# decadenza/SimpleStereo

Hardware: AMD Instinct MI355X
Metric: disparity MPixels/s (H*W*nDisp per second) (higher is better)
Workload: dtype f32

## Files before the change

### include/ssamd.h

```cpp
#ifndef SSAMD_H
#define SSAMD_H

#include <stdint.h>

#ifdef __cplusplus
extern "C" {
#endif

#define SSAMD_ABI_VERSION 8

#define SSAMD_OK 0
#define SSAMD_EINVAL (-1)
#define SSAMD_ENODEVICE (-2)
#define SSAMD_EHIP (-3)
#define SSAMD_ENOMEM (-4)
#define SSAMD_ELIMIT (-5)

int ssamd_abi_version(void);
const char *ssamd_last_error(void);
int ssamd_device_count(void);


int ssamd_asw(const uint8_t *img1, const uint8_t *img2, int height, int width,
              int winSize, int maxDisparity, int minDisparity,
// ... 83 lines not shown
                               int height, int width, int interpolation, int winSize, int maxDisparity, int minDisparity,
                               double gammaC, double gammaP, int consistent, int16_t *d_disparity, void *stream);

int ssamd_asw_exact_rectified_device(const uint8_t *d_raw1, const uint8_t *d_raw2, int src_height, int src_width,
                                     const float *d_mapx1, const float *d_mapy1, const float *d_mapx2, const float *d_mapy2,
                                     int height, int width, int interpolation, int winSize, int maxDisparity, int minDisparity,
                                     double gammaC, double gammaP, int consistent, int16_t *d_disparity, void *stream);

int ssamd_gsw_rectified_device(const uint8_t *d_raw1, const uint8_t *d_raw2, int src_height, int src_width,
                               const float *d_mapx1, const float *d_mapy1, const float *d_mapx2, const float *d_mapy2,
                               int height, int width, int interpolation, int winSize, int maxDisparity, int minDisparity,
                               int gamma, float fMax, int iterations, int bins, int16_t *d_disparity, void *stream);

int ssamd_reproject_device(const int16_t *d_disparity, int h, int w, const double *Q, float *d_points, void *stream);

int ssamd_iir_unwrap(const double *phase, int n, int h, int w, double tau, double *out, int device);
int ssamd_iir_unwrap_device(const double *d_phase, int n, int h, int w, double tau, double *d_out, void *stream);

int ssamd_np_unwrap(const double *p, long long outer, long long len, long long inner, double discont, double period, double *out,
                    int device);
int ssamd_np_unwrap_device(const double *d_p, long long outer, long long len, long long inner, double discont, double period,
                           double *d_out, void *stream);
int ssamd_np_unwrap_xy(const double *p, int n, int h, int w, double *out, int device);
int ssamd_np_unwrap_xy_device(const double *d_p, int n, int h, int w, double *d_out, void *stream);
int ssamd_np_unwrap_plan(long long outer, long long len, long long inner, int32_t *plan);

#define SSAMD_FTP_MAX_W 8192
int ssamd_ftp_phase(const uint8_t *img_obj, int ch_obj, const uint8_t *img_ref, int ch_ref, int h, int w, const double *fmin,
                    const double *fmax, int unwrap, double tau, double *out, int device);
int ssamd_ftp_phase_device(const uint8_t *d_img_obj, int ch_obj, const uint8_t *d_img_ref, int ch_ref, int h, int w,
                           const double *fmin, const double *fmax, int unwrap, double tau, double *d_out, void *stream);
int ssamd_ftp_band(int w, int h, const double *fmin, const double *fmax, int32_t *slo, int32_t *shi);


int ssamd_asw_costs(const uint8_t *img1, const uint8_t *img2, int height, int width,
                    int winSize, int maxDisparity, int minDisparity,
                    double gammaC, double gammaP, float *costs, int device);

int ssamd_asw_argmins(const uint8_t *img1, const uint8_t *img2, int height, int width,
                      int winSize, int maxDisparity, int minDisparity,
                      double gammaC, double gammaP,
                      int16_t *left_disparity, int16_t *right_match, int device);

int ssamd_bgr2lab(const uint8_t *img, int height, int width, float *lab, int device);

int ssamd_debug_libm(int which, int n, const void *in, void *out);
int ssamd_debug_exact_queue(int which, long long max_n, unsigned long long *entries, unsigned int *keys, long long *n);

int ssamd_debug_exact_costs(const uint8_t *img1, const uint8_t *img2, int height, int width, int winSize, double gammaC, double gammaP,
                            int n, const int *yxd, double *costs, double *lab1, double *lab2);

int ssamd_debug_gsw_sqrt(int n, float *out);

#define SSAMD_K_LAB 0
#define SSAMD_K_ASW_AGG 1
#define SSAMD_K_ASW_FIN 2
#define SSAMD_K_GSW_AGG 3
#define SSAMD_K_GSW_FIN 4
#define SSAMD_K_REMAP 5
#define SSAMD_K_REPROJECT 6
#define SSAMD_K_ASW_ALT 7
#define SSAMD_K_ASW_EXACT 8
#define SSAMD_K_UNWRAP 9
#define SSAMD_K_FTP 10
#define SSAMD_K_NPUNWRAP 11
#define SSAMD_K_COUNT 12
int ssamd_profile_enable(int on);
int ssamd_profile_reset(void);
int ssamd_profile_read(double *ms , long long *launches );
const char *ssamd_kernel_name(int slot);

int ssamd_set_option(const char *name, const char *value);

int ssamd_counter(int device, const char *name, long long *value);

int ssamd_autotune(int on);

int ssamd_asw_geometry(int width, int rows, int winSize, int maxDisparity, int minDisparity, int *out);

int ssamd_asw_kernel_form(int width, int rows, int winSize, int maxDisparity, int minDisparity, int *out);

int ssamd_gsw_geometry(int width, int rows, int winSize, int maxDisparity, int minDisparity, int *out);

#ifdef __cplusplus
}
#endif
#endif
```

### simplestereo_amd/_native.py

```python
import ctypes
import os

from .build import LIB_PATH as _DEFAULT_LIB_PATH

LIB_PATH = _DEFAULT_LIB_PATH
if os.environ.get("SSAMD_LIB"):
    if os.environ.get("SSAMD_EXPERIMENT") != "1":
        raise ImportError("SSAMD_LIB is an experiment hook: set SSAMD_EXPERIMENT=1 as well to load %s instead of the product "
                          "library" % os.environ["SSAMD_LIB"])
    LIB_PATH = os.environ["SSAMD_LIB"]
ABI_VERSION = 8

(K_LAB, K_ASW_AGG, K_ASW_FIN, K_GSW_AGG, K_GSW_FIN, K_REMAP, K_REPROJECT, K_ASW_ALT, K_ASW_EXACT, K_UNWRAP, K_FTP,
 K_NPUNWRAP, K_COUNT) = 0, 1, 2, 3, 4, 5, 6, 7, 8, 9, 10, 11, 12

_lib = None
_u8p = ctypes.c_void_p
_i16p = ctypes.c_void_p


class NativeError(RuntimeError):

    def __init__(self, code, msg):
        super().__init__("libssamd error %d: %s" % (code, msg))
# ... 46 lines not shown
    L.ssamd_gsw_device_rows2.restype = I
    L.ssamd_gsw_device_rows2.argtypes = [P, P, I, I, I, I, I, I, I, I, I, I, F, I, I, P, P]
    L.ssamd_asw_exact_device_rows2.restype = I
    L.ssamd_asw_exact_device_rows2.argtypes = [P, P, I, I, I, I, I, I, I, I, I, D, D, I, P, P]
    L.ssamd_asw_exact_rectified_device.restype = I
    L.ssamd_asw_exact_rectified_device.argtypes = [P, P, I, I, P, P, P, P, I, I, I, I, I, I, D, D, I, P, P]
    L.ssamd_asw_alternate.restype = I
    L.ssamd_asw_alternate.argtypes = [P, P, I, I, I, I, I, D, D, I, P, I]
    L.ssamd_asw_alternate_device.restype = I
    L.ssamd_asw_alternate_device.argtypes = [P, P, I, I, I, I, I, D, D, I, P, P]
    L.ssamd_asw_alternate_rows_device.restype = I
    L.ssamd_asw_alternate_rows_device.argtypes = [P, P, I, I, I, I, I, I, I, I, D, D, I, P, P]
    L.ssamd_asw_alternate_multi.restype = I
    L.ssamd_asw_alternate_multi.argtypes = [P, P, I, I, I, I, I, D, D, I, P, ctypes.POINTER(I), I]
    L.ssamd_asw_costs.restype = I
    L.ssamd_asw_costs.argtypes = [P, P, I, I, I, I, I, D, D, P, I]
    L.ssamd_asw_argmins.restype = I
    L.ssamd_asw_argmins.argtypes = [P, P, I, I, I, I, I, D, D, P, P, I]
    L.ssamd_bgr2lab.restype = I
    L.ssamd_bgr2lab.argtypes = [P, I, I, P, I]
    L.ssamd_remap_bgr_device.restype = I
    L.ssamd_remap_bgr_device.argtypes = [P, I, I, P, P, I, I, I, P, P]
    L.ssamd_reproject_device.restype = I
    L.ssamd_reproject_device.argtypes = [P, I, I, ctypes.POINTER(D), P, P]
    L.ssamd_iir_unwrap.restype = I
    L.ssamd_iir_unwrap.argtypes = [P, I, I, I, D, P, I]
    L.ssamd_iir_unwrap_device.restype = I
    L.ssamd_iir_unwrap_device.argtypes = [P, I, I, I, D, P, P]
    L.ssamd_ftp_phase.restype = I
    L.ssamd_ftp_phase.argtypes = [P, I, P, I, I, I, P, P, I, D, P, I]
    L.ssamd_ftp_phase_device.restype = I
    L.ssamd_ftp_phase_device.argtypes = [P, I, P, I, I, I, P, P, I, D, P, P]
    L.ssamd_ftp_band.restype = I
    L.ssamd_ftp_band.argtypes = [I, I, P, P, P, P]
    LL = ctypes.c_longlong
    L.ssamd_np_unwrap.restype = I
    L.ssamd_np_unwrap.argtypes = [P, LL, LL, LL, D, D, P, I]
    L.ssamd_np_unwrap_device.restype = I
    L.ssamd_np_unwrap_device.argtypes = [P, LL, LL, LL, D, D, P, P]
    L.ssamd_np_unwrap_xy.restype = I
    L.ssamd_np_unwrap_xy.argtypes = [P, I, I, I, P, I]
    L.ssamd_np_unwrap_xy_device.restype = I
    L.ssamd_np_unwrap_xy_device.argtypes = [P, I, I, I, P, P]
    L.ssamd_np_unwrap_plan.restype = I
    L.ssamd_np_unwrap_plan.argtypes = [LL, LL, LL, ctypes.POINTER(ctypes.c_int32)]
    L.ssamd_debug_exact_queue.restype = I
    L.ssamd_debug_exact_queue.argtypes = [I, ctypes.c_longlong, P, P, P]
    L.ssamd_debug_libm.restype = I
    L.ssamd_debug_libm.argtypes = [I, I, P, P]
    L.ssamd_debug_exact_costs.restype = I
    L.ssamd_debug_exact_costs.argtypes = [P, P, I, I, I, D, D, I, P, P, P, P]
    L.ssamd_debug_gsw_sqrt.restype = I
    L.ssamd_debug_gsw_sqrt.argtypes = [I, P]
    L.ssamd_profile_enable.restype = I
    L.ssamd_profile_enable.argtypes = [I]
    L.ssamd_profile_reset.restype = I
    L.ssamd_profile_read.restype = I
    L.ssamd_profile_read.argtypes = [ctypes.POINTER(D), ctypes.POINTER(ctypes.c_longlong)]
    L.ssamd_kernel_name.restype = ctypes.c_char_p
    L.ssamd_kernel_name.argtypes = [I]
    L.ssamd_autotune.restype = I
    L.ssamd_autotune.argtypes = [I]
    L.ssamd_asw_geometry.restype = I
    L.ssamd_asw_geometry.argtypes = [I, I, I, I, I, ctypes.POINTER(I)]
    L.ssamd_asw_kernel_form.restype = I
    L.ssamd_asw_kernel_form.argtypes = [I, I, I, I, I, ctypes.POINTER(I)]
    L.ssamd_gsw_geometry.restype = I
    L.ssamd_gsw_geometry.argtypes = [I, I, I, I, I, ctypes.POINTER(I)]
    L.ssamd_set_option.restype = I
    L.ssamd_set_option.argtypes = [ctypes.c_char_p, ctypes.c_char_p]
    L.ssamd_asw_rectified_device.restype = I
    L.ssamd_asw_rectified_device.argtypes = [P, P, I, I, P, P, P, P, I, I, I, I, I, I, D, D, I, P, P]
    L.ssamd_gsw_rectified_device.restype = I
    L.ssamd_gsw_rectified_device.argtypes = [P, P, I, I, P, P, P, P, I, I, I, I, I, I, I, F, I, I, P, P]
    L.ssamd_counter.restype = I
    L.ssamd_counter.argtypes = [I, ctypes.c_char_p, ctypes.POINTER(ctypes.c_longlong)]
    _lib = L
    return L


def set_option(name, value):
    check(lib().ssamd_set_option(name.encode(), None if value is None else str(value).encode()))


def counter(name, device=-1):
    v = ctypes.c_longlong(0)
    check(lib().ssamd_counter(device, name.encode(), ctypes.byref(v)))
    return int(v.value)


class options:

    def __init__(self, **kw):
        self.kw = kw

    def __enter__(self):
        done = []
        try:
            for k, v in self.kw.items():
                set_option(k, v)
                done.append(k)
        except Exception:
            for k in done:
                set_option(k, None)
            raise
        return self
# ... 47 lines not shown
```

### simplestereo_amd/csrc/asw_kernels.hip.h

```cpp
#pragma once
#include "common.hip.h"

namespace ssamd {

static constexpr int ASW_RX = 8;
static constexpr int ASW_RD = 4;
static constexpr int ASW_WB = 4;
static constexpr int ASW_MAX_THREADS = 768;
__host__ __device__ constexpr int asw_nwr(int rx) { return (rx + ASW_RD - 1 + 3) / 4 * 4; }
static_assert(ASW_RD == 4 && asw_nwr(8) == 12 && asw_nwr(4) == 8, "the main loop is unrolled for 8x4 and 4x4 register tiles");

struct AswGeom {
    int Tx, XG, DG, Dc, nchunks, threads;
    int Rx;
    int nL, nR, nRc, SR, Se, emask;
    int SL, hL, hR;
    int wseg, wlen;
    int JC;
    int e2;
    int e_bytes;
    int pipe;
    int NC, JCmax;
    int dephase;
    int wave_rx;
    int off_wL, off_wR, off_e, off_labL, off_labR, off_bgrL, off_bgrR, off_bestL, off_bestR, off_cen, off_prox;
    int lds_bytes;
    int lds_bytes_evol;
};

struct AswExactQueue {
    u64 *entries;
    uint32_t *ekeys;
    unsigned int *counter;
    unsigned char *flagL, *flagR;
    unsigned char *zeroL, *zeroR;
    unsigned char *zrow;
    unsigned int W;
    unsigned int cap;
    uint32_t tol;
    float sat_abs;
    uint32_t deep;
};

struct AswArgs {
    const PixRec *recL, *recR;
    const float *prox;
    u64 *keyL;
    u64 *keyR;
    int16_t *disp;
    const unsigned char *evol;
    int erow0, erows, evolW;
    float *costs;
    int cost_keys;
    int H, W, win, pad, minD, maxD, row0, rows;
    int ystep;
    int yb0;
    int yskip_at, yskip;
    float kC;
    AswExactQueue xq;
    AswGeom g;
    unsigned int *pq;
    int pq_nx, pq_ny, pq_items;
};
static constexpr int ASW_PQ_QUEUES = 8;
static constexpr int ASW_PQ_LINE = 32;

struct AswPipeTileId { int win, XG, DG, JC; };
__host__ __device__ constexpr int asw_cx_round_up(int v, int m) { return (v + m - 1) / m * m; }
__host__ __device__ constexpr int asw_cx_max(int a, int b) { return a > b ? a : b; }
__host__ __device__ constexpr AswGeom asw_pipe_geom_constexpr(AswPipeTileId t)
{
    AswGeom g{};
    const int win = t.win, p = win / 2;
    g.Rx = 8; g.JC = t.JC; g.pipe = 1; g.wave_rx = 0; g.e2 = 1; g.nchunks = 1;
    g.NC = (win + t.JC / 2) / t.JC;
    g.JCmax = asw_cx_max(t.JC, win - (g.NC - 1) * t.JC);
    g.XG = t.XG; g.DG = t.DG;
    g.Tx = 8 * t.XG; g.Dc = ASW_RD * t.DG;
    g.threads = asw_cx_round_up(t.XG * t.DG, 64);
    g.dephase = g.threads / 64 >= 12 ? 1 : 0;
    g.nL = g.Tx + 2 * p;
    g.nRc = g.Tx + g.Dc - 1;
    g.nR = g.nRc + 2 * p;
    g.hL = 0; g.hR = 0;
    g.SL = asw_cx_round_up(g.Tx, 4);
    g.SR = asw_cx_round_up(g.nRc + 1, 4);
    g.Se = 16 * ((t.DG + 3) / 4);
    g.emask = 0;
    const int wrows = 2 * g.JCmax;
    int off = 0;
    g.off_wL = off; off = (off + wrows * g.SL * 4 + 15) & ~15;
    g.off_wR = off; off = (off + wrows * g.SR * 4 + 15) & ~15;
    g.e_bytes = (g.nL * g.Se + 15) & ~15;
    g.off_e = off; off = (off + g.e_bytes * 2 + 15) & ~15;
    g.off_labL = off; off = (off + g.nL * 16 * 2 + 15) & ~15;
    g.off_labR = off; off = (off + g.nR * 16 * 2 + 15) & ~15;
    g.off_bestL = off; off = (off + g.Tx * 8 + 15) & ~15;
    g.off_bestR = off; off = (off + (g.nRc + 1) * 8 + 15) & ~15;
    g.off_cen = off; off = (off + (g.Tx + g.nRc) * 16 + 15) & ~15;
    g.off_prox = off; off = (off + win * 4 * 2 + 15) & ~15;
    g.lds_bytes_evol = off;
    g.off_bgrL = off; off = (off + g.nL * 4 * 2 + 15) & ~15;
    g.off_bgrR = off; off = (off + g.nR * 4 * 2 + 15) & ~15;
    g.lds_bytes = off;
    return g;
}
template <int SLC, int SRC, int SEC> struct AswPipeTile { static constexpr AswPipeTileId id{35, 1, 1, 16}; };
template <> struct AswPipeTile<120, 316, 208> { static constexpr AswPipeTileId id{35, 15, 49, 16}; };
template <> struct AswPipeTile<88, 348, 272> { static constexpr AswPipeTileId id{35, 11, 65, 16}; };
template <> struct AswPipeTile<216, 284, 80> { static constexpr AswPipeTileId id{35, 27, 17, 16}; };
inline bool asw_pipe_geom_matches(const AswGeom &a, const AswGeom &b)
{
    return a.pipe == b.pipe && a.Rx == b.Rx && a.JC == b.JC && a.NC == b.NC && a.JCmax == b.JCmax && a.XG == b.XG && a.DG == b.DG && a.Tx == b.Tx &&
           a.Dc == b.Dc && a.threads == b.threads && a.dephase == b.dephase && a.nL == b.nL && a.nRc == b.nRc && a.nR == b.nR && a.SL == b.SL &&
           a.SR == b.SR && a.Se == b.Se && a.e_bytes == b.e_bytes && a.off_wL == b.off_wL && a.off_wR == b.off_wR && a.off_e == b.off_e &&
// ... 577 lines not shown
```

### simplestereo_amd/csrc/asw_pipe_kernel.hip.h

```cpp
#pragma once
#include "asw_kernels.hip.h"
#ifndef SSAMD_KERNEL_TU
#include "lab_kernels.hip.h"
#endif

namespace ssamd {

#ifndef SSAMD_KERNEL_TU
static constexpr int TADV_COLS = 64;
template <bool BYTES>
__device__ __forceinline__ void asw_tad_tile(const void *__restrict__ srcL, const void *__restrict__ srcR, unsigned char *__restrict__ evol,
                                             int W, int pad, int minD, int Dc, int Se, int erow0, int erows, int evolW, int rd, long long npix_total,
                                             int bx, int by, int bz, char *smem)
{
    uint32_t *const sL = reinterpret_cast<uint32_t *>(smem);
    uint32_t *const sR = sL + TADV_COLS;
    const int r = erow0 + by, z = bz, uc0 = bx * TADV_COLS;
    const int P = Se >> 2, dlo = minD + z * Dc, dhi = dlo + Dc - 1;
    const int u0 = uc0 - pad, xr0 = u0 - dhi;
    auto pixel = [&](const void *src, int col) -> uint32_t {
        const size_t q = (size_t)r * W + col;
        if constexpr (BYTES) {
            typedef uint32_t __attribute__((aligned(1))) u32_unaligned;
            const uint8_t *const b = reinterpret_cast<const uint8_t *>(src) + 3 * q;
            return (long long)q + 1 < npix_total ? (*reinterpret_cast<const u32_unaligned *>(b) & 0xffffffu)
                                                 : ((uint32_t)b[0] | ((uint32_t)b[1] << 8) | ((uint32_t)b[2] << 16));
        } else {
            return reinterpret_cast<const PixRec *>(src)[q].bgrx;
        }
    };
    for (int k = threadIdx.x; k < 2 * TADV_COLS + Dc; k += blockDim.x) {
        const bool isL = k < TADV_COLS;
        const int col = isL ? u0 + k : xr0 + (k - TADV_COLS);
        const uint32_t v = (unsigned)col < (unsigned)W ? pixel(isL ? srcL : srcR, col) : 0x80000000u;
        (isL ? sL : sR)[isL ? k : k - TADV_COLS] = v;
    }
    __syncthreads();
    const int ncols = min(TADV_COLS, evolW - uc0);
    uint32_t *const out = reinterpret_cast<uint32_t *>(evol + (((size_t)z * erows + by) * (size_t)evolW + uc0) * Se);
    auto dword = [&](int c, int slot, uint32_t lp) {
        uint32_t v = 0;
        const int d0 = rd == 6 ? 6 * (slot >> 1) + 4 * (slot & 1) : 4 * slot, nv = rd == 6 && (slot & 1) ? 2 : 4;
        if (!(lp >> 31) && d0 < Dc) {
            const uint32_t *const rp = sR + c + (Dc - 1) - d0;
#pragma unroll
            for (int q = 0; q < 4; ++q) {
                const uint32_t rv = q < nv && d0 + q < Dc ? rp[-q] : 0x80000000u;
                if (!(rv >> 31)) v |= min(__builtin_amdgcn_sad_u8(lp, rv, 0u), 40u) << (8 * q);
            }
        }
        return v;
    };
    if ((P & 3) == 0) {
        const int P4 = P >> 2;
// ... 62 lines not shown

template <bool WITH_COSTS, int SLC = 0, int SRC = 0, int SEC = 0, bool CG = false>
__global__ __launch_bounds__(ASW_MAX_THREADS, 3) void asw_aggregate_pipe_kernel(const AswArgs A0)
{
    constexpr bool STATIC = SLC > 0;
    static_assert(!CG || STATIC, "compile-time geometry belongs to a static tile");
    constexpr int RX = ASW_RX;
    constexpr int NWR = asw_nwr(RX);
    extern __shared__ __attribute__((aligned(16))) char smem[];
    constexpr AswGeom SG = asw_pipe_geom_constexpr(AswPipeTile<SLC, SRC, SEC>::id);
    static_assert(!STATIC || (SG.SL == SLC && SG.SR == SRC && SG.Se == SEC), "the strides name the tile");
    uint32_t *const pq_next = reinterpret_cast<uint32_t *>(smem + (CG ? SG : A0.g).off_prox);
    int pq_q = 0;
    auto run_item = [&](const AswArgs &A, const int ibx, const int iby, const int ibz, const int inx) __attribute__((always_inline)) {
    const bool persist = A.pq != nullptr;
    const AswGeom &g = CG ? SG : A.g;
    float *const wL = reinterpret_cast<float *>(smem + g.off_wL);
    float *const wR = reinterpret_cast<float *>(smem + g.off_wR);
    unsigned char *const eT0 = reinterpret_cast<unsigned char *>(smem + g.off_e);
    float4 *const labL = reinterpret_cast<float4 *>(smem + g.off_labL);
    float4 *const labR = reinterpret_cast<float4 *>(smem + g.off_labR);
    uint32_t *const bgrL = reinterpret_cast<uint32_t *>(smem + g.off_bgrL);
    uint32_t *const bgrR = reinterpret_cast<uint32_t *>(smem + g.off_bgrR);
    u64 *const bestL = reinterpret_cast<u64 *>(smem + g.off_bestL);
    u64 *const bestR = reinterpret_cast<u64 *>(smem + g.off_bestR);
    float4 *const cenLab = reinterpret_cast<float4 *>(smem + g.off_cen);

    const int tid = threadIdx.x, nthr = blockDim.x;
    const int W = A.W, win = CG ? AswPipeTile<SLC, SRC, SEC>::id.win : A.win, p = CG ? AswPipeTile<SLC, SRC, SEC>::id.win / 2 : A.pad;
    const int Tx = g.Tx, Dc = g.Dc, nL = g.nL, nR = g.nR, nRc = g.nRc, SR = g.SR, Se = g.Se;
    const int JC = g.JC, NC = g.NC;
    size_t Wz = (size_t)W;
    asm volatile("" : "+s"(Wz));
    int bx = ibx;
    if ((inx & 7) == 0) bx = (bx & 7) * (inx >> 3) + (bx >> 3);
    const int x0 = bx * Tx;
    const int y = asw_out_row(A, iby);
    const int dlo = A.minD + ibz * Dc;
    const int dhi = dlo + Dc - 1;
    if (min(x0 + Tx - 1, W - 1) - dlo < 0) {
        if (A.disp)
            for (int k = threadIdx.x; k < Tx && x0 + k < W; k += blockDim.x)
                A.disp[(size_t)(y - A.row0) * Wz + x0 + k] = (int16_t)(x0 + k);
        if (persist) {
            if (threadIdx.x == 0) *pq_next = atomicAdd(A.pq + pq_q * ASW_PQ_LINE, 1u);
            __syncthreads();
        }
        return;
    }
    uint32_t pq_ticket = 0;
    if (persist && threadIdx.x == 0) pq_ticket = atomicAdd(A.pq + pq_q * ASW_PQ_LINE, 1u);
    const int segL_lo = x0 - p, xrc_lo = x0 - dhi, segR_lo = xrc_lo - p;
    const int phase = g.dephase ? __builtin_amdgcn_readfirstlane((int)(threadIdx.x >> 8)) : 1;

    float accN[RX][ASW_RD], accS[RX][ASW_RD];
#pragma unroll
    for (int a = 0; a < RX; ++a)
#pragma unroll
        for (int b = 0; b < ASW_RD; ++b) { accN[a][b] = 0.f; accS[a][b] = 0.f; }

    for (int k = tid; k < Tx; k += nthr) bestL[k] = KEY_NONE;
    for (int k = tid; k <= nRc; k += nthr) bestR[k] = KEY_NONE;
    for (int c = tid; c < Tx + nRc; c += nthr) {
        const bool isL = c < Tx;
        const int ccol = isL ? x0 + c : xrc_lo + (c - Tx);
        float4 v = make_float4(0.f, 0.f, 0.f, 0.f);
        if ((unsigned)ccol < (unsigned)W) {
            const PixRec q = (isL ? A.recL : A.recR)[(size_t)y * Wz + ccol];
            v = make_float4(q.L, q.a, q.b, 1.f);
        }
        cenLab[c] = v;
    }

    const int i_lo = max(0, p - y), i_hi = min(win, A.H + p - y);

    auto stage_row = [&](int i) {
        int tids = threadIdx.x;
        asm volatile("" : "+v"(tids));
        const int buf = i & 1, r = y - p + i;
        const PixRec *const rowL = A.recL + (size_t)r * Wz;
        const PixRec *const rowR = A.recR + (size_t)r * Wz;
        for (int k = tids; k < nL + nR; k += nthr) {
            const bool isL = k < nL;
            const int idx = isL ? k : k - nL;
            const int col = (isL ? segL_lo : segR_lo) + idx;
            PixRec v;
            v.L = __builtin_inff();
            v.a = v.b = 0.f;
            v.bgrx = 0u;
            if ((unsigned)col < (unsigned)W) v = (isL ? rowL : rowR)[col];
            (isL ? labL + buf * nL : labR + buf * nR)[idx] = make_float4(v.L, v.a, v.b, 0.f);
            if (!A.evol) (isL ? bgrL + buf * nL : bgrR + buf * nR)[idx] = v.bgrx;
        }
    };
    auto build_e = [&](int i, int t_lo, int t_hi) {
        int tidb = threadIdx.x;
        asm volatile("" : "+v"(tidb));
        unsigned char *const eT = eT0 + (i & 1) * g.e_bytes;
        const uint32_t *const bgrLc = bgrL + (i & 1) * nL, *const bgrRc = bgrR + (i & 1) * nR;
        const int e_q = nthr / nL, e_r = nthr - e_q * nL;
        int t = t_lo + tidb;
        int sp = t / nL, ul = t - sp * nL;
        while (t < t_hi) {
            const uint32_t lp = bgrLc[ul];
            const uint32_t *const rp = bgrRc + (ul + (Dc - 1) - 8 * sp);
            uint32_t lo = 0, hi = 0;
// ... 30 lines not shown
        constexpr int NTHR = STATIC ? asw_cx_round_up((SLC / ASW_RX) * ((SRC - SLC) / ASW_RD), 64) : 0;
        static_assert(!STATIC || (SG.Tx == SLC && SG.nRc == SRC - 1 && SG.threads == NTHR), "the strides name the centres and the threads");
        const int TxB = STATIC ? SLC : Tx, nRcB = STATIC ? SRC - 1 : nRc, nw = (STATIC ? NTHR : nthr) >> 6;
        const int nLw = (TxB + 63) >> 6, ncw = nLw + ((nRcB + 63) >> 6);
        const float4 *const labLc = labL + (i & 1) * nL, *const labRc = labR + (i & 1) * nR;
        cfloat *const prow = reinterpret_cast<cfloat *>(reinterpret_cast<uintptr_t>(A.prox)) + i * win;
        auto batch = [&](auto n_, const float4 &cen, const float4 *sp, cfloat *pp, float *wp, int stride) {
            constexpr int N = decltype(n_)::value;
            float4 tp[N];
            float pr[N], wv[N];
#pragma unroll
            for (int u = 0; u < N; ++u) { tp[u] = sp[u]; pr[u] = pp[u]; }
#pragma unroll
            for (int u = 0; u < N; ++u) {
                asm volatile("" ::"v"(tp[u].w));
                const float dL = tp[u].x - cen.x, da = tp[u].y - cen.y, db = tp[u].z - cen.z;
                wv[u] = fmaf(db, db, fmaf(da, da, dL * dL));
            }
#pragma unroll
            for (int u = 0; u < N; ++u) wv[u] = __builtin_amdgcn_sqrtf(wv[u]);
#pragma unroll
            for (int u = 0; u < N; ++u) wv[u] = asw_weight_finish(wv[u], A.kC, pr[u]);
#pragma unroll
            for (int u = 0; u < N; ++u) wp[u * stride] = wv[u];
        };
        auto build_side = [&](auto left_, int cc, int jb_t, int je_t) {
            constexpr bool LEFT = decltype(left_)::value;
            const int stride = LEFT ? (STATIC ? SLC : g.SL) : (STATIC ? SRC : SR);
            if (cc >= (LEFT ? TxB : nRcB)) return;
            const float4 cen = cenLab[(LEFT ? 0 : TxB) + cc];
            asm volatile("" ::"v"(cen.w));
            const float4 *sp = (LEFT ? labLc : labRc) + cc + jb_t;
            cfloat *pp = prow + jb_t;
            float *wp = (LEFT ? wL : wR) + cc + (rb + jb_t - jb) * stride;
            int j = jb_t;
#pragma nounroll
            for (; j + ASW_WB <= je_t; j += ASW_WB, sp += ASW_WB, pp += ASW_WB, wp += ASW_WB * stride)
                batch(std::integral_constant<int, ASW_WB>{}, cen, sp, pp, wp, stride);
            const int rem = je_t - j;
            if (rem == 1) batch(std::integral_constant<int, 1>{}, cen, sp, pp, wp, stride);
            else if (rem == 2) batch(std::integral_constant<int, 2>{}, cen, sp, pp, wp, stride);
            else if (rem == 3) batch(std::integral_constant<int, 3>{}, cen, sp, pp, wp, stride);
        };
        int full = 0;
        while (full + nw <= ncw) full += nw;
        const int rest = ncw - full;
        int slen = je - jb, nseg = 1;
        if (rest > 0 && full > 0) {
            int per = 0;
            for (int a = rest; a <= nw; a += rest) ++per;
            for (slen = ASW_WB; slen * per < je - jb;) slen += ASW_WB;
            while (nseg * slen < je - jb) ++nseg;
        }
        for (int t = wave; t < full + rest * nseg; t += nw) {
            int cw = t, jb_t = jb, je_t = je;
            if (t >= full && nseg > 1) {
                int q = t - full, sgm = 0;
                while (q >= rest) { q -= rest; ++sgm; }
                cw = full + q;
                jb_t = jb + sgm * slen;
                je_t = min(je, jb_t + slen);
            }
            if (cw < nLw) build_side(std::true_type{}, 64 * cw + lane, jb_t, je_t);
            else build_side(std::false_type{}, 64 * (cw - nLw) + lane, jb_t, je_t);
        }
    };
    auto chunk_end = [&](int c) { return c == NC - 1 ? win : (c + 1) * JC; };
    const int nE = nL * ((g.DG + 1) >> 1);
    auto build_next = [&](int i, int c, int cb) {
        const bool more_rows = i + 1 < i_hi;
        if (c == 0 && more_rows) stage_row(i + 1);
        if (c == 0 && more_rows && A.evol) load_e(i + 1);
        if (c + 1 < NC || more_rows) {
            const int cn = c + 1 < NC ? c + 1 : 0;
            build_weights(c + 1 < NC ? i : i + 1, cn * JC, chunk_end(cn), (cb ^ 1) * g.JCmax);
        }
        if (c >= 1 && more_rows && !A.evol) build_e(i + 1, (int)((long long)nE * (c - 1) / (NC - 1)), (int)((long long)nE * c / (NC - 1)));
    };

    stage_row(i_lo);
    if (persist && threadIdx.x == 0) *pq_next = pq_ticket;
    if (A.evol) load_e(i_lo);
    __syncthreads();
    if (!A.evol) build_e(i_lo, 0, nE);
    build_weights(i_lo, 0, chunk_end(0), 0);

    const int DGe = max(1, min(g.DG, (min(min(x0 + Tx, W) - 1, x0 + Tx - 1) - dlo) / ASW_RD + 1));
    const int nact = g.XG * DGe;
    int pk_xd;
    bool run;
    {
        const int tidm = threadIdx.x;
        int xg, dg;
        const int F = DGe >> 4, Lo = DGe & 15, nfull = g.XG * F;
        const int grp16 = tidm >> 4, r16 = tidm & 15;
        if (grp16 < nfull) {
            xg = grp16 / F;
            int gi = grp16 - xg * F;
            if (xg & 1) gi = F - 1 - gi;
            dg = 16 * gi + r16;
        } else {
            const int q = tidm - 16 * nfull;
            xg = Lo ? q / Lo : g.XG;
            dg = 16 * F + (Lo ? q - xg * Lo : 0);
        }
        pk_xd = xg | (dg << 16);
        const bool tile_live = tidm < nact && x0 + RX * xg < W && dlo + ASW_RD * dg <= A.maxD &&
                               x0 + RX * xg + RX - 1 - (dlo + ASW_RD * dg) >= 0;
        run = __builtin_amdgcn_ballot_w64(tile_live) != 0 && tidm < nact;
    }

    int cb = 0;
#pragma nounroll
    for (int i = i_lo; i < i_hi; ++i) {
        const unsigned char *const eT = eT0 + (i & 1) * g.e_bytes;
        AswRow ew[RX];

#pragma nounroll
        for (int c = 0; c < NC; ++c) {
            __syncthreads();
            const int jc = c * JC, jend = chunk_end(c);
            const int rb = cb * g.JCmax;
            if (phase == 0) build_next(i, c, cb);
            if (run) {
                const int xg = pk_xd & 0xffff, dg = pk_xd >> 16;
                const unsigned char *erow = eT + (RX * xg + (jc == 0 ? 0 : RX - 1 + jc)) * Se + 4 * dg;
                if (jc == 0) {
#pragma unroll
                    for (int n = 0; n < RX - 1; ++n) {
                        asw_row_unpack(ew[n], *reinterpret_cast<const uint32_t *>(erow));
                        erow += Se;
                    }
                }
                const float *wlp = wL + rb * g.SL + 8 * xg;
                const float *wrp = wR + rb * SR + (RX * xg - ASW_RD * dg + Dc - ASW_RD);
                for (int j0 = jc; j0 < jend; j0 += RX) {
#define SSAMD_PSTEP(JJ)                                                                             \
    if (j0 + (JJ) < jend) {                                                                         \
        const uint32_t epk = *reinterpret_cast<const uint32_t *>(erow + (STATIC ? (JJ) * SEC : 0)); \
        if constexpr (!STATIC) erow += Se;                                                          \
        float wl[RX], wr[NWR];                                                                      \
        {                                                                                           \
            const float *const wl_ = wlp + (STATIC ? (JJ) * SLC : 0);                              \
            const float *const wr_ = wrp + (STATIC ? (JJ) * SRC : 0);                              \
            const float4 v0 = *reinterpret_cast<const float4 *>(wl_);                              \
            wl[0] = v0.x; wl[1] = v0.y; wl[2] = v0.z; wl[3] = v0.w;                                 \
            const float4 v1 = *reinterpret_cast<const float4 *>(wl_ + 4);                          \
            wl[4] = v1.x; wl[5] = v1.y; wl[6] = v1.z; wl[7] = v1.w;                                 \
            const float4 r0 = *reinterpret_cast<const float4 *>(wr_);                              \
            const float4 r1 = *reinterpret_cast<const float4 *>(wr_ + 4);                          \
            const float4 r2 = *reinterpret_cast<const float4 *>(wr_ + 8);                          \
            asm volatile("" ::"v"(r2.w));       \
            wr[0] = r0.x; wr[1] = r0.y; wr[2] = r0.z; wr[3] = r0.w;                                 \
            wr[4] = r1.x; wr[5] = r1.y; wr[6] = r1.z; wr[7] = r1.w;                                 \
            wr[8] = r2.x; wr[9] = r2.y; wr[10] = r2.z; wr[11] = r2.w;                               \
        }                                                                                           \
        if constexpr (!STATIC) { wlp += g.SL; wrp += SR; }                                         \
               \
        _Pragma("unroll") for (int xi = 0; xi < RX; ++xi) {                                         \
            if (xi == RX - 1) asw_row_unpack(ew[((JJ) + RX - 1) % RX], epk);                        \
            const AswRow &row_ = ew[((JJ) + xi) % RX];                                              \
            _Pragma("unroll") for (int di = 0; di < ASW_RD; ++di) {                                 \
                const float w_ = wl[xi] * wr[xi - di + ASW_RD - 1];                                 \
// ... 71 lines not shown
```

### simplestereo_amd/csrc/ssamd_api.hip

```cpp
#include <hip/hip_runtime.h>

#include <algorithm>
#include <array>
#include <atomic>
#include <list>
#include <map>
#include <thread>
#include <cmath>
#include <cstdarg>
#include <cstdio>
#include <cstdlib>
#include <cstring>
#include <mutex>
#include <string>
#include <vector>

#include "../../include/ssamd.h"
#include "asw_kernels.hip.h"
#include "asw_pipe_kernel.hip.h"
#include "asw_wave_kernel.hip.h"
#include "asw_wave6_kernel.hip.h"
#include "asw_alt_kernels.hip.h"
namespace ssamd {
#define SSAMD_PIPE_INSTANCE(C, SL, SR, SE) extern template __global__ void asw_aggregate_pipe_kernel<C, SL, SR, SE>(const AswArgs);
// ... 832 lines not shown
        }
    }
    const long long items = per_row * rows_main;
    long long workers = r.t.asw_persist > 0 ? std::min<long long>(r.t.asw_persist, slots) : (r.t.asw_persist < 0 && items >= 64 * slots ? slots : 0);
    workers = std::min(workers, items);
    if (workers > 0 && items < (1ll << 30)) {
        const size_t pq_bytes = (size_t)(ASW_PQ_QUEUES + 1) * ASW_PQ_LINE * 4;
        if (!c.pq.ptr) {
            if (int prc = c.pq.reserve(pq_bytes)) return prc;
            HIP_TRY(hipMemsetAsync(c.pq.ptr, 0, pq_bytes, r.s));
        }
        HIP_TRY(hipMemsetAsync(c.pq.ptr, 0, (size_t)ASW_PQ_QUEUES * ASW_PQ_LINE * 4, r.s));
        AswArgs pa = a;
        pa.pq = (unsigned int *)c.pq.ptr;
        pa.pq_nx = (int)grid.x; pa.pq_ny = rows_main; pa.pq_items = (int)items;
        ++c.persist_launches;
        hipLaunchKernelGGL(pk, dim3((unsigned)workers), dim3(g.threads), pipe_lds, r.s, pa);
    } else {
        hipLaunchKernelGGL(pk, dim3(grid.x, rows_main, grid.z), dim3(g.threads), pipe_lds, r.s, a);
    }
    HIP_TRY(hipGetLastError());
    if (rows_main < r.grows) {
        ++c.tail_splits;
        AswArgs t = a;
        t.g = tail_g;
        t.yb0 = rows_main;
        const AswKernel tk = asw_pick_pipe_kernel(c, tail_g, r.win, r.d_costs != nullptr, 0);
        const int tail_lds = a.evol ? tail_g.lds_bytes_evol : tail_g.lds_bytes;
        if (int grc = grant_dyn_lds(c, (const void *)tk, tail_lds)) return grc;
        hipLaunchKernelGGL(tk, dim3((r.W + tail_g.Tx - 1) / tail_g.Tx, r.grows - rows_main, tail_g.nchunks), dim3(tail_g.threads),
                           tail_lds, r.s, t);
        HIP_TRY(hipGetLastError());
    }
    return SSAMD_OK;
}

int asw_launch(AswRun &r, const AswGeom &g)
{
    r.geom = g;
    if (g.wave_rx) {
        AswWaveArgs wa;
        asw_fill_args(wa, r, g);
        wa.g = r.wave;
        const AswWaveKernel wk = asw_pick_wave_kernel(wa.g, r.d_costs != nullptr, r.t.wave_unroll != 0);
        const int lds = wa.g.wave_lds * wa.g.waves, xt = (r.W + wa.g.Txw - 1) / wa.g.Txw;
        if (int grc = grant_dyn_lds(r.c, (const void *)wk, lds)) return grc;
        hipLaunchKernelGGL(wk, dim3((xt + wa.g.waves - 1) / wa.g.waves, r.grows, 1), dim3(64 * wa.g.waves), lds, r.s, wa);
        HIP_TRY(hipGetLastError());
        return SSAMD_OK;
    }
    AswArgs a{};
    asw_fill_args(a, r, g);
    a.g = g;
    const dim3 grid((r.W + g.Tx - 1) / g.Tx, r.grows, g.nchunks);
    if (g.pipe) return asw_launch_pipe(r, a, grid);
    const bool chunked = g.JC < r.win;
    AswKernel kern = chunked ? (r.d_costs ? asw_aggregate_kernel<true, true> : asw_aggregate_kernel<false, true>)
                             : (r.d_costs ? asw_aggregate_kernel<true, false> : asw_aggregate_kernel<false, false>);
    if (g.Rx == 4)
        kern = chunked ? (r.d_costs ? asw_aggregate_kernel<true, true, 4> : asw_aggregate_kernel<false, true, 4>)
                       : (r.d_costs ? asw_aggregate_kernel<true, false, 4> : asw_aggregate_kernel<false, false, 4>);
    if (int grc = grant_dyn_lds(r.c, (const void *)kern, g.lds_bytes)) return grc;
    hipLaunchKernelGGL(kern, grid, dim3(g.threads), g.lds_bytes, r.s, a);
    HIP_TRY(hipGetLastError());
    return SSAMD_OK;
}

int asw_autotune(AswRun &r)
{
    hipStream_t s = r.s;
    hipEvent_t e0 = nullptr, e1 = nullptr;
    HIP_TRY(hipEventCreate(&e0));
    HIP_TRY(hipEventCreate(&e1));
    bool all_prepared = true;
    const bool want_evol = r.t.asw_evol != 0;
    for (const AswGeom &g : r.trial) {
        if (asw_prepare_volume(r, g) != SSAMD_OK) { all_prepared = false; continue; }
        if (g.pipe && !g.wave_rx && want_evol && !r.evol) all_prepared = false;
        if (asw_launch(r, g) != SSAMD_OK) all_prepared = false;
    }
    const int fastest = autotune_rounds(r.trial.size(), 4, false, e0, e1, s, &all_prepared, [&](size_t ci) {
        const AswGeom &g = r.trial[ci];
        const bool launched = asw_prepare_volume(r, g) == SSAMD_OK && asw_launch(r, g) == SSAMD_OK;
        if (g.pipe && !g.wave_rx && want_evol && !r.evol) all_prepared = false;
        return launched;
    });
    if (fastest >= 0) r.geom = r.trial[fastest];
    (void)hipEventDestroy(e0);
    (void)hipEventDestroy(e1);
    if (all_prepared) autotune_keep(g_asw_geom, r.shape, r.geom);
    else g_err.clear();
    return SSAMD_OK;
}

int asw_final_volume(AswRun &r, AswGeom &final_geom)
{
    int rc = asw_prepare_volume(r, final_geom);
    if (rc == SSAMD_ENOMEM && final_geom.wave_rx) {
        ++r.c.evol_fallbacks;
        g_err.clear();
        final_geom.wave_rx = 0;
        r.geom = final_geom;
        if (!asw_is_direct(r, final_geom) && !r.need_keys) {
            if ((rc = reset_keys(r.c.keyL, r.nout, r.s))) return rc;
            r.need_keys = true;
        }
// ... 1081 lines not shown
    *n = 0;
    if (!c->xflags.ptr || c->exact_calls == 0) return SSAMD_OK;
    HIP_TRY(hipDeviceSynchronize());
    unsigned int ctr[5] = {0, 0, 0, 0, 0};
    HIP_TRY(hipMemcpy(ctr, c->xflags.ptr, sizeof(ctr), hipMemcpyDeviceToHost));
    const unsigned int cnt = which ? ctr[4] : ctr[0], cap = which ? c->xrawcap : c->xcap;
    *n = cnt;
    const size_t m = (size_t)std::min<long long>(std::min<unsigned int>(cnt, cap), max_n);
    if (m == 0) return SSAMD_OK;
    const void *src = which ? c->xraw.ptr : c->xqueue.ptr;
    if (!src) return SSAMD_OK;
    HIP_TRY(hipMemcpy(entries, src, m * 8, hipMemcpyDeviceToHost));
    if (which && keys) HIP_TRY(hipMemcpy(keys, (const char *)src + (size_t)c->xrawcap * 8, m * 4, hipMemcpyDeviceToHost));
    return SSAMD_OK;
}

int ssamd_debug_libm(int which, int n, const void *in, void *out)
{
    if (!in || !out || n < 0 || which < 0 || which > 3)
        return fail(SSAMD_EINVAL, "ssamd_debug_libm: which = 0 (exp, doubles), 1 (powf(x, 1/3), floats), 2 (sqrt, doubles), 3 (x / 0.7 + x / 5.0, doubles)");
    if (n == 0) return SSAMD_OK;
    CtxLock c;
    int rc = get_ctx(-1, c);
    if (rc) return rc;
    const size_t bytes = (size_t)n * (which == 1 ? 4 : 8);
    if ((rc = c->lab.reserve(2 * bytes))) return rc;
    char *const d_in = (char *)c->lab.ptr, *const d_out = d_in + bytes;
    HIP_TRY(hipMemcpyAsync(d_in, in, bytes, hipMemcpyHostToDevice, c->stream));
    hipLaunchKernelGGL(debug_libm_kernel, dim3((n + 255) / 256), dim3(256), 0, c->stream, which, n, (const void *)d_in, (void *)d_out);
    HIP_TRY(hipGetLastError());
    HIP_TRY(hipMemcpyAsync(out, d_out, bytes, hipMemcpyDeviceToHost, c->stream));
    HIP_TRY(hipStreamSynchronize(c->stream));
    return SSAMD_OK;
}

int ssamd_debug_gsw_sqrt(int n, float *out)
{
    int what = 0;
    if (n < 0) { what = 1; n = -n; }
    if (!out || n <= 0 || n > GSW_TAB_SIZE) return fail(SSAMD_EINVAL, "bad argument");
    CtxLock c;
    int rc = get_ctx(-1, c);
    if (rc) return rc;
    if ((rc = c->lab.reserve((size_t)n * 4))) return rc;
    hipStream_t s = c->stream;
    ScratchOrder order(*c, s);
    hipLaunchKernelGGL(gsw_sqrt_probe_kernel, dim3((n + 255) / 256), dim3(256), 0, s, (float *)c->lab.ptr, n, what);
    HIP_TRY(hipGetLastError());
    HIP_TRY(hipMemcpyAsync(out, c->lab.ptr, (size_t)n * 4, hipMemcpyDeviceToHost, s));
    HIP_TRY(hipStreamSynchronize(s));
    return SSAMD_OK;
}

int ssamd_profile_enable(int on)
{
    for (auto &c : g_ctx) {
        std::lock_guard<std::mutex> lk(c.mu);
        c.prof.on = on != 0;
    }
    return SSAMD_OK;
}

int ssamd_profile_reset(void)
{
    DeviceGuard guard;
    for (auto &c : g_ctx) {
        std::lock_guard<std::mutex> lk(c.mu);
        if (c.dev < 0) continue;
        (void)hipSetDevice(c.dev);
        c.prof.drain();
        std::fill(c.prof.ms, c.prof.ms + SSAMD_K_COUNT, 0.0);
        std::fill(c.prof.n, c.prof.n + SSAMD_K_COUNT, 0LL);
    }
    return SSAMD_OK;
}

int ssamd_profile_read(double *ms, long long *launches)
{
    DeviceGuard guard;
    for (int k = 0; k < SSAMD_K_COUNT; ++k) { if (ms) ms[k] = 0; if (launches) launches[k] = 0; }
    for (auto &c : g_ctx) {
        std::lock_guard<std::mutex> lk(c.mu);
        if (c.dev < 0) continue;
        (void)hipSetDevice(c.dev);
        c.prof.drain();
        for (int k = 0; k < SSAMD_K_COUNT; ++k) { if (ms) ms[k] += c.prof.ms[k]; if (launches) launches[k] += c.prof.n[k]; }
    }
    return SSAMD_OK;
}

}
```

### simplestereo_amd/csrc/ssamd_options.h

```cpp
#pragma once

#define SSAMD_OPTIONS(X) \
    X("SSAMD_ASW_GEOM", asw_geom, std::string, "", v, !x.empty())    \
    X("SSAMD_GSW_GEOM", gsw_geom, std::string, "", v, false) \
    X("SSAMD_ASW_PIPE", asw_pipe, int, -1, atoi(v), x >= 0)    \
    X("SSAMD_ASW_DEPHASE", asw_dephase, int, -1, atoi(v), x >= 0)    \
    X("SSAMD_ASW_EVOL", asw_evol, int, 1, atoi(v), x != 1)    \
    X("SSAMD_ASW_WAVE", asw_wave, int, -1, atoi(v) != 0 ? 1 : 0, x >= 0)    \
    X("SSAMD_ASW_WAVE_RX", wave_rx, int, 0, atoi(v), x != 0)    \
    X("SSAMD_ASW_WAVE_WG", wave_wg, int, 0, std::max(1, std::min(4, atoi(v))), x != 0)    \
    X("SSAMD_ASW_WAVE_UNROLL", wave_unroll, int, 1, atoi(v), false)    \
    X("SSAMD_ASW_WAVE_MERGE", wave_merge, int, 1, atoi(v), x != 1)    \
    X("SSAMD_ASW_STATIC", asw_static, int, 1, atoi(v), x != 1)    \
    X("SSAMD_ASW_EVOL_MAX_MB", evol_max_mb, int, 0, std::max(0, atoi(v)), x != 0)    \
    X("SSAMD_ASW_WAVE_RD", wave_rd, int, 0, atoi(v), x != 0)    \
    X("SSAMD_ASW_NO_E2", no_e2, bool, false, true, x) \
    X("SSAMD_ASW_XOR_ONLY", xor_only, bool, false, true, x) \
    X("SSAMD_MULTI_ALLOW_REPEAT", multi_allow_repeat, bool, false, true, false) \
    X("SSAMD_ALT_QUEUE_CAP", alt_queue_cap, int, 0, std::max(1, atoi(v)), false)    \
    X("SSAMD_AUTOTUNE", autotune_env, int, -2, atoi(v) > 0 ? 1 : (atoi(v) < 0 ? -1 : 0), false)    \
    X("SSAMD_ASW_EVOL_FAIL", evol_fail, int, 0, atoi(v), false)    \
    X("SSAMD_ASW_TAIL", asw_tail, int, -1, atoi(v), false)    \
    X("SSAMD_ASW_PERSIST", asw_persist, int, -1, atoi(v), x > 0)    \
    X("SSAMD_ASW_WAVE_CREG", wave_creg, int, 1, atoi(v), x != 1)    \
    X("SSAMD_ASW_LDS_RELAX", lds_relax, int, 1, atoi(v), x != 1)    \
    X("SSAMD_ASW_PREPASS_FUSE", prepass_fuse, int, 1, atoi(v), false)    \
    X("SSAMD_EXACT_TOL", exact_tol, int, 128, std::max(0, atoi(v)), false)    \
    X("SSAMD_EXACT_CAP", exact_cap, int, 0, std::max(1, atoi(v)), false)    \
    X("SSAMD_EXACT_RAWCAP", exact_rawcap, int, 0, std::max(1, atoi(v)), false)    \
    X("SSAMD_UNWRAP_ROWS", unwrap_rows, int, 0, std::max(0, std::min(UNWRAP_MAX_ROWS, atoi(v))), false)

struct Tuning {
#define X(NAME, MEMBER, TYPE, UNSET, PARSE, FORCES) TYPE MEMBER = UNSET;
    SSAMD_OPTIONS(X)
#undef X
};

bool tuning_assign(Tuning &t, const std::string &name, const char *v)
{
#define X(NAME, MEMBER, TYPE, UNSET, PARSE, FORCES) \
    if (name == NAME) { if (v) t.MEMBER = PARSE; else t.MEMBER = UNSET; return true; }
    SSAMD_OPTIONS(X)
#undef X
    return false;
}

const char *const kTuningNames[] = {
#define X(NAME, MEMBER, TYPE, UNSET, PARSE, FORCES) NAME,
    SSAMD_OPTIONS(X)
#undef X
};

bool asw_geometry_forced(const Tuning &t)
{
#define X(NAME, MEMBER, TYPE, UNSET, PARSE, FORCES) { const TYPE &x = t.MEMBER; (void)x; if (FORCES) return true; }
    SSAMD_OPTIONS(X)
#undef X
    return false;
}
```

Baseline: 10720.

## Pack live border tiles densely and rotate weight-build waves in ASW pipe kernel

```diff
diff --git a/include/ssamd.h b/include/ssamd.h
--- a/include/ssamd.h
+++ b/include/ssamd.h
@@ -159,6 +159,9 @@
 
 int ssamd_debug_gsw_sqrt(int n, float *out);
 
+int ssamd_debug_pipe_deal(int XG, int DG, int width, int minDisparity, int maxDisparity, int tile, int chunk, int border, int n,
+                          int *xg, int *dg, int *nact);
+
 #define SSAMD_K_LAB 0
 #define SSAMD_K_ASW_AGG 1
 #define SSAMD_K_ASW_FIN 2
diff --git a/simplestereo_amd/_native.py b/simplestereo_amd/_native.py
--- a/simplestereo_amd/_native.py
+++ b/simplestereo_amd/_native.py
@@ -122,6 +122,8 @@
     L.ssamd_debug_exact_costs.argtypes = [P, P, I, I, I, D, D, I, P, P, P, P]
     L.ssamd_debug_gsw_sqrt.restype = I
     L.ssamd_debug_gsw_sqrt.argtypes = [I, P]
+    L.ssamd_debug_pipe_deal.restype = I
+    L.ssamd_debug_pipe_deal.argtypes = [I, I, I, I, I, I, I, I, I, P, P, P]
     L.ssamd_profile_enable.restype = I
     L.ssamd_profile_enable.argtypes = [I]
     L.ssamd_profile_reset.restype = I
diff --git a/simplestereo_amd/csrc/asw_kernels.hip.h b/simplestereo_amd/csrc/asw_kernels.hip.h
--- a/simplestereo_amd/csrc/asw_kernels.hip.h
+++ b/simplestereo_amd/csrc/asw_kernels.hip.h
@@ -61,6 +61,7 @@
     AswGeom g;
     unsigned int *pq;
     int pq_nx, pq_ny, pq_items;
+    int border;
 };
 static constexpr int ASW_PQ_QUEUES = 8;
 static constexpr int ASW_PQ_LINE = 32;
diff --git a/simplestereo_amd/csrc/asw_pipe_deal.h b/simplestereo_amd/csrc/asw_pipe_deal.h
--- /dev/null
+++ b/simplestereo_amd/csrc/asw_pipe_deal.h
@@ -0,0 +1,57 @@
+#pragma once
+
+namespace ssamd {
+
+__host__ __device__ constexpr int asw_deal_min(int a, int b) { return a < b ? a : b; }
+__host__ __device__ constexpr int asw_deal_max(int a, int b) { return a > b ? a : b; }
+
+__host__ __device__ __forceinline__ int asw_pipe_live_groups(int xg, int DG, int x0, int W, int dlo, int maxD)
+{
+    const int xl = x0 + 8 * xg;
+    if (xl >= W) return 0;
+    const int m = asw_deal_min(maxD, xl + 7) - dlo;
+    return m < 0 ? 0 : asw_deal_min(DG, (m >> 2) + 1);
+}
+
+__host__ __device__ __forceinline__ int asw_pipe_deal_dge(int DG, int Tx, int x0, int W, int dlo)
+{
+    return asw_deal_max(1, asw_deal_min(DG, (asw_deal_min(asw_deal_min(x0 + Tx, W) - 1, x0 + Tx - 1) - dlo) / 4 + 1));
+}
+
+__host__ __device__ __forceinline__ int asw_pipe_deal_rect(int tid, int XG, int DGe)
+{
+    int xg, dg;
+    const int F = DGe >> 4, Lo = DGe & 15, nfull = XG * F;
+    const int grp16 = tid >> 4, r16 = tid & 15;
+    if (grp16 < nfull) {
+        xg = grp16 / F;
+        int gi = grp16 - xg * F;
+        if (xg & 1) gi = F - 1 - gi;
+        dg = 16 * gi + r16;
+    } else {
+        const int q = tid - 16 * nfull;
+        xg = Lo ? q / Lo : XG;
+        dg = 16 * F + (Lo ? q - xg * Lo : 0);
+    }
+    return xg | (dg << 16);
+}
+
+__host__ __device__ __forceinline__ int asw_pipe_live_tiles(int XG, int DG, int x0, int W, int dlo, int maxD)
+{
+    int s = 0;
+    for (int k = 0; k < XG; ++k) s += asw_pipe_live_groups(k, DG, x0, W, dlo, maxD);
+    return s;
+}
+
+__host__ __device__ __forceinline__ int asw_pipe_deal_dense(int tid, int XG, int DG, int x0, int W, int dlo, int maxD)
+{
+    int xg = 0, base = 0, end = 0;
+    for (int k = 0; k < XG; ++k) {
+        end += asw_pipe_live_groups(k, DG, x0, W, dlo, maxD);
+        if (tid >= end) { xg = k + 1; base = end; }
+    }
+    if (xg >= XG) { xg = XG; base = tid; }
+    return xg | ((tid - base) << 16);
+}
+
+}
diff --git a/simplestereo_amd/csrc/asw_pipe_kernel.hip.h b/simplestereo_amd/csrc/asw_pipe_kernel.hip.h
--- a/simplestereo_amd/csrc/asw_pipe_kernel.hip.h
+++ b/simplestereo_amd/csrc/asw_pipe_kernel.hip.h
@@ -1,5 +1,6 @@
 #pragma once
 #include "asw_kernels.hip.h"
+#include "asw_pipe_deal.h"
 #ifndef SSAMD_KERNEL_TU
 #include "lab_kernels.hip.h"
 #endif
@@ -168,6 +169,7 @@
     if (persist && threadIdx.x == 0) pq_ticket = atomicAdd(A.pq + pq_q * ASW_PQ_LINE, 1u);
     const int segL_lo = x0 - p, xrc_lo = x0 - dhi, segR_lo = xrc_lo - p;
     const int phase = g.dephase ? __builtin_amdgcn_readfirstlane((int)(threadIdx.x >> 8)) : 1;
+    int build_rot = 0;
 
     float accN[RX][ASW_RD], accS[RX][ASW_RD];
 #pragma unroll
@@ -304,7 +306,9 @@
             for (slen = ASW_WB; slen * per < je - jb;) slen += ASW_WB;
             while (nseg * slen < je - jb) ++nseg;
         }
-        for (int t = wave; t < full + rest * nseg; t += nw) {
+        int t0 = wave;
+        if (build_rot > 0 && build_rot + ncw <= nw) t0 = wave >= build_rot ? wave - build_rot : wave - build_rot + nw;
+        for (int t = t0; t < full + rest * nseg; t += nw) {
             int cw = t, jb_t = jb, je_t = je;
             if (t >= full && nseg > 1) {
                 int q = t - full, sgm = 0;
@@ -337,30 +341,22 @@
     if (!A.evol) build_e(i_lo, 0, nE);
     build_weights(i_lo, 0, chunk_end(0), 0);
 
-    const int DGe = max(1, min(g.DG, (min(min(x0 + Tx, W) - 1, x0 + Tx - 1) - dlo) / ASW_RD + 1));
-    const int nact = g.XG * DGe;
+    const int DGe = asw_pipe_deal_dge(g.DG, Tx, x0, W, dlo);
+    const int nlive = A.border ? asw_pipe_live_tiles(g.XG, g.DG, x0, W, dlo, A.maxD) : g.XG * DGe;
+    const bool dense = nlive < g.XG * DGe;
+    const int nact = dense ? nlive : g.XG * DGe;
     int pk_xd;
     bool run;
     {
         const int tidm = threadIdx.x;
-        int xg, dg;
-        const int F = DGe >> 4, Lo = DGe & 15, nfull = g.XG * F;
-        const int grp16 = tidm >> 4, r16 = tidm & 15;
-        if (grp16 < nfull) {
-            xg = grp16 / F;
-            int gi = grp16 - xg * F;
-            if (xg & 1) gi = F - 1 - gi;
-            dg = 16 * gi + r16;
-        } else {
-            const int q = tidm - 16 * nfull;
-            xg = Lo ? q / Lo : g.XG;
-            dg = 16 * F + (Lo ? q - xg * Lo : 0);
-        }
-        pk_xd = xg | (dg << 16);
+        if (dense) pk_xd = asw_pipe_deal_dense(tidm, g.XG, g.DG, x0, W, dlo, A.maxD);
+        else pk_xd = asw_pipe_deal_rect(tidm, g.XG, DGe);
+        const int xg = pk_xd & 0xffff, dg = pk_xd >> 16;
         const bool tile_live = tidm < nact && x0 + RX * xg < W && dlo + ASW_RD * dg <= A.maxD &&
                                x0 + RX * xg + RX - 1 - (dlo + ASW_RD * dg) >= 0;
         run = __builtin_amdgcn_ballot_w64(tile_live) != 0 && tidm < nact;
     }
+    if (A.border) build_rot = (nact + 63) >> 6;
 
     int cb = 0;
 #pragma nounroll
diff --git a/simplestereo_amd/csrc/ssamd_api.hip b/simplestereo_amd/csrc/ssamd_api.hip
--- a/simplestereo_amd/csrc/ssamd_api.hip
+++ b/simplestereo_amd/csrc/ssamd_api.hip
@@ -908,6 +908,7 @@
     AswArgs a{};
     asw_fill_args(a, r, g);
     a.g = g;
+    a.border = r.t.asw_border != 0;
     const dim3 grid((r.W + g.Tx - 1) / g.Tx, r.grows, g.nchunks);
     if (g.pipe) return asw_launch_pipe(r, a, grid);
     const bool chunked = g.JC < r.win;
@@ -2095,6 +2096,28 @@
     return SSAMD_OK;
 }
 
+int ssamd_debug_pipe_deal(int XG, int DG, int width, int minDisparity, int maxDisparity, int tile, int chunk, int border, int n, int *xg, int *dg, int *nact)
+{
+    if (XG < 1 || DG < 1 || XG > 4096 || DG > 4096 || width < 1 || minDisparity < 0 || maxDisparity < minDisparity || tile < 0 || chunk < 0 ||
+        n < 0 || (n > 0 && (!xg || !dg)) || !nact)
+        return fail(SSAMD_EINVAL, "bad argument");
+    const int Tx = ASW_RX * XG, x0 = tile * Tx, dlo = minDisparity + chunk * ASW_RD * DG;
+    if (x0 >= width || dlo > maxDisparity) return fail(SSAMD_EINVAL, "no such tile or disparity chunk");
+    if (std::min(x0 + Tx - 1, width - 1) - dlo < 0) {
+        *nact = 0;
+        return SSAMD_OK;
+    }
+    const int DGe = asw_pipe_deal_dge(DG, Tx, x0, width, dlo);
+    const int nlive = border ? asw_pipe_live_tiles(XG, DG, x0, width, dlo, maxDisparity) : XG * DGe;
+    const bool dense = nlive < XG * DGe;
+    *nact = dense ? nlive : XG * DGe;
+    for (int tid = 0; tid < n; ++tid) {
+        const int pk = dense ? asw_pipe_deal_dense(tid, XG, DG, x0, width, dlo, maxDisparity) : asw_pipe_deal_rect(tid, XG, DGe);
+        xg[tid] = pk & 0xffff; dg[tid] = pk >> 16;
+    }
+    return SSAMD_OK;
+}
+
 int ssamd_profile_enable(int on)
 {
     for (auto &c : g_ctx) {
diff --git a/simplestereo_amd/csrc/ssamd_options.h b/simplestereo_amd/csrc/ssamd_options.h
--- a/simplestereo_amd/csrc/ssamd_options.h
+++ b/simplestereo_amd/csrc/ssamd_options.h
@@ -22,6 +22,7 @@
     X("SSAMD_ASW_EVOL_FAIL", evol_fail, int, 0, atoi(v), false)    \
     X("SSAMD_ASW_TAIL", asw_tail, int, -1, atoi(v), false)    \
     X("SSAMD_ASW_PERSIST", asw_persist, int, -1, atoi(v), x > 0)    \
+    X("SSAMD_ASW_BORDER", asw_border, int, 1, atoi(v), false)    \
     X("SSAMD_ASW_WAVE_CREG", wave_creg, int, 1, atoi(v), x != 1)    \
     X("SSAMD_ASW_LDS_RELAX", lds_relax, int, 1, atoi(v), x != 1)    \
     X("SSAMD_ASW_PREPASS_FUSE", prepass_fuse, int, 1, atoi(v), false)    \
```

Result: no change. 10720 (median of 2 runs) (+0.0%).
